# y2w-oc/CMR-Agent

Measured on AMD Instinct MI355X. Metric: registration iters/sec (KITTI 352x1216 img + 16384 pts, 1 geo forward + 10 agent steps), higher is better.
Workload: dtype f32; 1 GPU; BASELINE.json configs[1]: KittiConfig, batch 8 per GPU, 16384 pts, 352x1216 image, 10 agent steps, fp32, hash-filled weights; batch_per_gpu=8, parallelism=batch sharding, no data-path collective

## Files before the change

cmr_agent_amd/models/CMRAgent.py:

```python
import torch
import torch.nn as nn

from .. import ops
from ..utils.streams import fork_join
from . import _pack
from ._pack import Planned
from .ImageResNet import to_nhwc
from .PointNN import ConvBNReLURes1D

SLOPE = 0.01


def _mlp(sizes):
    layers = []
    for i in range(len(sizes) - 1):
        layers.append(nn.Linear(sizes[i], sizes[i + 1]))
        if i < len(sizes) - 2:
            layers.append(nn.LeakyReLU(inplace=True))
    return nn.Sequential(*layers)


class CMRAgent(Planned):
    def __init__(self, config):
        super().__init__()
# ... 47 lines not shown
                e[f:, :] = torch.eye(f, dtype=w1.dtype, device=w1.device)
                ent.update(wsca=None, wscb=e, b2=q["b2f"])
            p["s3d"].append(ent)
        return p

    def _embed_3d(self, state3d_rows, B, N):
        p = self.plan()
        layers = self.state_3d_embed
        q0 = layers[0].plan()
        r = ops.cbr_block(state3d_rows, q0["l1"][0], q0["l1"][1], q0["l2"][0], q0["b2f"], q0["sc"][0], 0.2,
                          rows_per_batch=N, want_colmax="partials")
        if r is None:
            return None
        feat, part = r
        for i, ent in enumerate(p["s3d"]):
            glue = ops.colmax_bias2(part, B, N // 32, ent["w1b"], ent["b1"], ent["wscb"], ent["b2"])
            if glue is not None:
                b1b, b2b = glue[0], glue[1]
            else:
                g = ops.colmax_partials(part, B, N // 32)
                b1b = ops.linear(g, ent["w1b"], ent["b1"])
                b2b = ops.linear(g, ent["wscb"], ent["b2"])
            last = i == 2
            r = ops.cbr_block(feat, ent["w1a"], b1b, ent["w2"], b2b, ent["wsca"], 0.2, rows_per_batch=N,
                              want_y=not last, want_colmax="partials")
            if r is None:
                return None
            feat, part = r
        return ops.colmax_partials(part, B, N // 32)

    FUSED_TAIL = True
    TAIL_T = True

    def _embed_2d(self, state2d, B, split):
        p = self.plan()
        c = 2 * self.config.embed_dim
        x = state2d
        for stage, ((wa, ba, ua), (wb, bb, ub)) in enumerate(p["convs"]):
            if stage == 0 and split is not None:
                img_src, proj, cache = split
                tag = (id(self), id(p))
                if cache.get("tag") != tag:
                    wi, bi, ui = p["conv0_img"]
                    cache["val"] = ops.conv3x3(img_src, wi, bi, c, 1, 1.0, u=ui)
                    cache["tag"] = tag
                wp, _, up = p["conv0_proj"]
                x = ops.conv3x3(proj, wp, None, c, 1, SLOPE, res=cache["val"], u=up, out_bf16=True)
            else:
                x = ops.conv3x3(x, wa, ba, c, 1, SLOPE, u=ua, out_bf16=True)
            x = ops.conv3x3(x, wb, bb, c, 1, SLOPE, pool=2 if stage < 3 else 1, u=ub, out_bf16=stage < 3)
            if stage == 3:
                kh, kw = self.config.image_H // 8, self.config.image_W // 8
                if (x.shape[1], x.shape[2]) != (kh, kw):
                    raise ValueError("state_2d is %dx%d at the global pool, config says %dx%d" % (x.shape[1], x.shape[2], kh, kw))
        return x

    def _embed_3d_any(self, state3d_rows, B, N):
        e3d = self._embed_3d(state3d_rows, B, N)
        if e3d is None:
            layers = self.state_3d_embed
            feat = layers[0].rows(state3d_rows)
            for i in (1, 2, 3):
                g = ops.colmax(feat, B, N)
                feat = layers[i].rows(feat, x2=g, div2=N)
            e3d = ops.colmax(feat, B, N)
        return e3d

    def forward_cl(self, state2d, state3d_rows, B, N, split=None):
        self._require_eval()
        e3d, e2d = fork_join(lambda: self._embed_3d_any(state3d_rows, B, N), lambda: self._embed_2d(state2d, B, split), tag="agent")
        p = self.plan()
        _, kh, kw, c = e2d.shape
        xr = e2d.view(B * kh * kw, c)
        heads = [p[name] for name in ("policy_r", "policy_t", "value")]
        if self.FUSED_TAIL and e3d.is_contiguous():
            if self.TAIL_T and p["tail_t"]:
                out, acts = ops.agent_heads_t(xr, B, kh * kw, p["c24t"], p["c26t"], e3d, [p[name + "_t"] for name in ("policy_r", "policy_t", "value")],
                                              SLOPE, actions=(self.config.num_steps, self.degree_r, self.degree_t))
# ... 72 lines not shown
```

cmr_agent_amd/models/IMGPCEnDecoder.py:

```python
import math

import torch
import torch.nn as nn

from .. import ops
from ..utils.streams import fork_join
from ._pack import Planned
from .ImageResNet import ResidualBlock
from .IMGPCEncoder import IMGPCEncoder
from .LinearAttention import LinearAttention
from .PointNN import ConvBNReLURes1D, bcl_from_rows


def position_encoding_sine_2d(d_model, h, w):
    pe = torch.zeros((d_model, h, w))
    y_pos = torch.ones((h, w)).cumsum(0).float().unsqueeze(0)
    x_pos = torch.ones((h, w)).cumsum(1).float().unsqueeze(0)
    div = torch.exp(torch.arange(0, d_model // 2, 2).float() * (-math.log(10000.0) / (d_model // 2)))[:, None, None]
    pe[0::4], pe[1::4] = torch.sin(x_pos * div), torch.cos(x_pos * div)
    pe[2::4], pe[3::4] = torch.sin(y_pos * div), torch.cos(y_pos * div)
    return pe.permute(1, 2, 0).contiguous()


class IMGPCEnDecoder(Planned):
    def __init__(self, config):
        super().__init__()
        self.config = config
        self.encoder = IMGPCEncoder(config)
        self.H_proxy = config.image_H // config.patch_size
        self.W_proxy = config.image_W // config.patch_size
        self.img_proxy_num = self.H_proxy * self.W_proxy
        self.pt_sample_num = config.pt_sample_num
        f = config.embed_dim
        self.node_fuse_convs = nn.ModuleList([ConvBNReLURes1D(2 * f, f)] +
                                             [ConvBNReLURes1D(f, f) for _ in range(config.node_fuse_res_num - 1)] +
                                             [nn.Dropout(0.1)])
        la = lambda: nn.ModuleList([LinearAttention(d_model=f, nhead=config.LA_head_num)
                                    for _ in range(config.linear_attention_num)])
        self.node_self_LA, self.pixel_to_node_LA, self.node_to_pixel_LA, self.pixel_self_LA = la(), la(), la(), la()
        self.img_fuse_convs = nn.ModuleList([ResidualBlock(2 * f, f)] +
                                            [ResidualBlock(f, f) for _ in range(config.img_fuse_res_num - 1)] +
                                            [nn.Dropout(0.1)])

    def _build_plan(self):
        return {"pe": {}}

    def _pos_table(self, h, w, device):
        cache = self.plan()["pe"]
        if (h, w) not in cache:
            cache[(h, w)] = position_encoding_sine_2d(self.config.embed_dim, h, w).to(device)
        return cache[(h, w)]

    def forward_cl(self, data_batch):
        self._require_eval()
        cl = self.encoder.forward_cl(data_batch)
        B, geo, f2 = cl["B"], cl["geo"], cl["f2"]
        _, h, w, f = f2.shape
        P = self.config.patch_size
        def fuse_nodes():
            nod = self.node_fuse_convs[0].rows(cl["node_feat"], x2=cl["pt_proxy"], idx2=cl["node2proxy_global"])
            for layer in list(self.node_fuse_convs)[1:-1]:
                nod = layer.rows(nod)
            return nod

        def fuse_pixels():
            x = ops.upsample_concat(f2, cl["img_proxy"], P)
            for i, layer in enumerate(list(self.img_fuse_convs)[:-1]):
                x = layer.forward_cl(x, post=self._pos_table(h, w, x.device) if i == 0 else None)
            return x

        nod, x = fork_join(fuse_nodes, fuse_pixels, tag="fuse")
        cl["vis_feat"] = x
        pix = x.view(B * h * w, f)
        M, L = geo.M, h * w
        for i in range(self.config.linear_attention_num):
            nod = self.pixel_to_node_LA[i].rows(nod, pix, B, M, L)
            pix = self.node_to_pixel_LA[i].rows(pix, nod, B, L, M)
            n0, p0 = nod, pix
            nod, pix = fork_join(lambda: self.node_self_LA[i].rows(n0, n0, B, M, M),
                                 lambda: self.pixel_self_LA[i].rows(p0, p0, B, L, L), tag="fine_sa")
        cl["fused_img_feat"] = pix.view(B, h, w, f)
        cl["fused_node_feat"] = nod
        cl["h"], cl["w"] = h, w
        return cl

    @staticmethod
    def publish(data_batch, cl):
        IMGPCEncoder.publish(data_batch, cl)
        data_batch['vis_feat'] = cl["vis_feat"].permute(0, 3, 1, 2)
        data_batch['fused_img_feat'] = cl["fused_img_feat"].permute(0, 3, 1, 2)
        data_batch['fused_node_feat'] = bcl_from_rows(cl["fused_node_feat"], cl["B"])

    def forward(self, data_batch):
        cl = self.forward_cl(data_batch)
        self.publish(data_batch, cl)
        data_batch['_cmr'] = cl
        return 0
```

cmr_agent_amd/models/IMGPCEncoder.py:

```python
import torch
import torch.nn as nn

from .. import ops
from ..utils.streams import fork_join, in_side_branch as streams_in_side_branch
import os
TOWERS_SWAPPED = os.environ.get("CMR_TOWERS_SWAPPED", "0") == "1"
from ._pack import Planned, device_of
from ._vit import Attention, Block, Mlp
from .ImageViT import ImageTransformer
from .PointNN import bcl_from_rows
from .PointViT import PointGeometry, PointTransformer


class IMGPCEncoder(Planned):
    def __init__(self, config):
        super().__init__()
        self.config = config
        self.pt_transformer = PointTransformer(config)
        self.img_transformer = ImageTransformer(config)
        n = config.num_ca_layer_coarse
        self.i2p_ca_layers = nn.ModuleList([Block(config) for _ in range(n)])
        self.p2i_ca_layers = nn.ModuleList([Block(config) for _ in range(n)])
        self.pt_sa_layers = nn.ModuleList([Block(config) for _ in range(n)])
        self.img_sa_layers = nn.ModuleList([Block(config) for _ in range(n)])

    def _build_plan(self):
        return {}

    def forward_cl(self, data_batch):
        dev = device_of(self)
        img = data_batch['img'].to(dev).contiguous()
        pc = data_batch['pc'].to(dev)
        node = data_batch['node'].to(dev)
        idx = data_batch['pt2node'].to(dev)
        B, Q = pc.shape[0], self.config.num_proxy

        def point_tower():
            geo = PointGeometry(pc, node, idx)
            return (geo,) + tuple(self.pt_transformer.forward_cl(geo))

        def image_tower():
            budget = ops.TOWER_CU_BUDGET if ops.CONV_BF16 else ops.TOWER_CU_BUDGET_F32
            if budget:
                give = (256 - budget) * (26.1 * pc.shape[2] / float(img.shape[2] * img.shape[3])) ** 2
                budget = 256 - 8 * int(min(256 - budget, give) / 8 + 0.5)
            if budget and budget < 256:
                with ops.conv_cu_budget(budget):
                    return self.img_transformer.forward_cl(img)
            if not ops.CONV_BF16 and ops.TOWER_SLICES_F32 > 1:
                with ops.conv_slices(ops.TOWER_SLICES_F32):
                    return self.img_transformer.forward_cl(img)
            return self.img_transformer.forward_cl(img)

        if TOWERS_SWAPPED and torch.cuda.is_available() and not streams_in_side_branch():
            (img_proxy, T, f2, f1, f0), (geo, pt_proxy, n2p, n2p_global, pt_feat, node_feat) = fork_join(image_tower, point_tower, tag="towers",
                                                                                                       main_first=False)
        else:
            (geo, pt_proxy, n2p, n2p_global, pt_feat, node_feat), (img_proxy, T, f2, f1, f0) = fork_join(point_tower, image_tower, tag="towers")
        for i in range(self.config.num_ca_layer_coarse):
            img_proxy = self.p2i_ca_layers[i].rows(img_proxy, pt_proxy, B, T, Q)
            pt_proxy = self.i2p_ca_layers[i].rows(pt_proxy, img_proxy, B, Q, T)
            ip, pp = img_proxy, pt_proxy
            pt_proxy, img_proxy = fork_join(lambda: self.pt_sa_layers[i].rows(pp, None, B, Q, Q),
                                            lambda: self.img_sa_layers[i].rows(ip, None, B, T, T), tag="coarse_sa")
        return dict(geo=geo, B=B, T=T, Q=Q, pc=pc, f2=f2, f1=f1, f0=f0, img_proxy=img_proxy, pt_proxy=pt_proxy,
                    node2proxy=n2p, node2proxy_global=n2p_global, pt_feat=pt_feat, node_feat=node_feat)

    @staticmethod
    def publish(data_batch, cl):
        B = cl["B"]
        nchw = lambda f: f.permute(0, 3, 1, 2)
        data_batch['pc_i'] = cl["pc"]
        data_batch['img_feat_2'], data_batch['img_feat_1'], data_batch['img_feat_0'] = nchw(cl["f2"]), nchw(cl["f1"]), nchw(cl["f0"])
        data_batch['node2proxy'] = cl["node2proxy"]
        data_batch['pt_feat'] = bcl_from_rows(cl["pt_feat"], B)
        data_batch['node_feat'] = bcl_from_rows(cl["node_feat"], B)
        data_batch['img_proxy'] = cl["img_proxy"].view(B, cl["T"], -1)
        data_batch['pt_proxy'] = cl["pt_proxy"].view(B, cl["Q"], -1)
        data_batch['pc'] = cl["pc"]

    def forward(self, data_batch):
        cl = self.forward_cl(data_batch)
        self.publish(data_batch, cl)
        data_batch['_cmr'] = cl
        return 0
```

cmr_agent_amd/models/ImageResNet.py:

```python
import torch
import torch.nn as nn

from .. import ops
from . import _pack
from ._pack import Planned


def _conv_bn(cin, cout, k, stride, pad):
    return [nn.Conv2d(cin, cout, k, stride, pad), nn.BatchNorm2d(cout)]


class ResidualBlock(Planned):
    SLOPE = 0.2

    def __init__(self, inchannel=3, outchannel=3, stride=1):
        super().__init__()
        assert stride in (1, 2)
        self.inchannel, self.outchannel, self.stride = inchannel, outchannel, stride
        self.conv_layers = nn.Sequential(*_conv_bn(inchannel, inchannel, 3, stride, 1),
                                         nn.LeakyReLU(self.SLOPE, inplace=True),
                                         *_conv_bn(inchannel, outchannel, 3, 1, 1))
        self.final_relu = nn.LeakyReLU(self.SLOPE, inplace=True)
        if stride == 2:
            self.shortcut = nn.Sequential(*_conv_bn(inchannel, outchannel, 3, 2, 1))
# ... 16 lines not shown
            p.update(stem=True, wa=wa.contiguous(), ba=ba.contiguous(), w3=w3.reshape(co, 27).t().contiguous(),
                     w1=w1.reshape(co, 3).t().contiguous(), bb=(b3 + b1).contiguous())
            return p
        p["stem"] = False
        p["a"] = _pack.conv9(cl[0], cl[1])
        p["b"] = _pack.conv9(cl[3], cl[4])
        if isinstance(self.shortcut, nn.Identity):
            p["sc"] = None
        elif self.shortcut[0].kernel_size == (1, 1):
            p["sc"] = ("1x1",) + _pack.lin(self.shortcut[0], self.shortcut[1])
        else:
            p["sc"] = ("3x3",) + _pack.conv9(self.shortcut[0], self.shortcut[1])
        return p

    def forward_cl(self, x, post=None, out_bf16=False):
        self._require_eval()
        p = self.plan()
        if p["stem"]:
            assert post is None
            return ops.stem_block(x, p["wa"], p["ba"], p["w3"], p["w1"], p["bb"], self.SLOPE, out_bf16=out_bf16)
        t = ops.conv3x3(x, p["a"][0], p["a"][1], self.inchannel, self.stride, self.SLOPE, u=p["a"][2],
                        out_bf16=post is None and getattr(p["b"][2], "bf16", None) is not None)
        sc = p["sc"]
        xb = x.dtype == torch.bfloat16
        if sc is None:
            res = x
        elif sc[0] == "1x1":
            B, H, W, c = x.shape
            res = ops.linear(x.view(B * H * W, c), sc[1], sc[2]).view(B, H, W, self.outchannel)
        else:
            res = ops.conv3x3(x, sc[1], sc[2], self.outchannel, 2, 1.0, u=sc[3], out_bf16=xb)
        return ops.conv3x3(t, p["b"][0], p["b"][1], self.outchannel, 1, self.SLOPE, res=res, post=post, u=p["b"][2], out_bf16=out_bf16)

    def forward(self, x):
        if self.inchannel == 3:
            return self.forward_cl(x.contiguous()).permute(0, 3, 1, 2)
        return self.forward_cl(to_nhwc(x)).permute(0, 3, 1, 2)


def to_nhwc(x):
    xp = x.permute(0, 2, 3, 1)
    if xp.is_contiguous():
        return xp
    B, C, H, W = x.shape
    return ops.transpose(x.contiguous().view(B, C, H * W)).view(B, H, W, C)


class MiniResNet(Planned):

    def __init__(self, inchannel=3, outchannel=3):
        super().__init__()
        strides = (1, 1, 2, 1, 2, 1)
        self.residual_learning = nn.ModuleList(
            [ResidualBlock(inchannel if i == 0 else outchannel, outchannel, s) for i, s in enumerate(strides)])

    def _build_plan(self):
        return {}

    def forward_cl(self, img_nchw):
        rl = self.residual_learning
        st = bool(ops.CONV_BF16 and ops.BF16_STORE and ops.BF16_CHAINS and self._bf16_served())
        x = rl[0].forward_cl(img_nchw, out_bf16=st)
        f0 = rl[1].forward_cl(x, out_bf16=st)
        f1 = rl[3].forward_cl(rl[2].forward_cl(f0, out_bf16=st), out_bf16=st)
        f2 = rl[5].forward_cl(rl[4].forward_cl(f1))
        return f2, f1, f0
# ... 13 lines not shown
```

cmr_agent_amd/ops.py:

```python
import collections
import math
import os

import numpy as np
import torch

from . import _lib

ACT_NONE, ACT_RELU, ACT_LRELU, ACT_GELU, ACT_ELU1 = 0, 1, 2, 3, 4
f32 = torch.float32
GRID_Y_MAX = 65535


def _stream():
    return torch.cuda.current_stream().cuda_stream


def _p(t):
    return None if t is None else t.data_ptr()


def _rows(t, name="tensor"):
    if t.dim() != 2 or t.stride(1) != 1 or t.dtype != f32 or not t.is_cuda:
        raise ValueError("%s must be a 2-D float32 device tensor with unit inner stride, got %s %s %s" % (
# ... 110 lines not shown

def colmax_bias2(part, B, tiles_per_batch, w1, b1, w2, b2, want_g=False):
    C = part.shape[1]
    n1, n2 = w1.shape[0], w2.shape[0]
    if COLMAX_BIAS2 == "0" or (COLMAX_BIAS2 == "fp32" and CONV_BF16) or C != 64 or n1 % 4 or n2 % 4 or not (w1.is_contiguous() and w2.is_contiguous()) or w1.shape[1] != C or w2.shape[1] != C:
        return None
    y1 = torch.empty((B, n1), dtype=f32, device=part.device)
    y2 = torch.empty((B, n2), dtype=f32, device=part.device)
    g = torch.empty((B, C), dtype=f32, device=part.device) if want_g else None
    rc = _lib.call("cmr_colmax_bias2_f32", _p(part), B, int(tiles_per_batch), C, _p(w1), _p(b1), n1, _p(w2), _p(b2), n2, _p(g), _p(y1), _p(y2), _stream(),
                   allow_unsupported=True)
    return None if rc == _lib.UNSUPPORTED else (y1, y2, g)


def layernorm64(x, gamma, beta, eps, res=None, out=None):
    _rows(x, "x")
    if out is None:
        out = torch.empty((x.shape[0], 64), dtype=f32, device=x.device)
    _lib.call("cmr_layernorm64_f32", _p(x), _ld(x), _p(gamma), _p(beta), float(eps), _p(res),
              _ld(res) if res is not None else 0, _p(out), _ld(out), x.shape[0], _stream())
    return out


CONV_BF16 = False
BF16_CHAINS = True
BF16_STORE = True
STRIDE2_FRAGS = True
WINOGRAD = True
WINO_MIN_TILES = 64


TOWER_CU_BUDGET = 160
TOWER_CU_BUDGET_F32 = 0


TOWER_SLICES_F32 = int(os.environ.get("CMR_TOWER_SLICES", "1"))


import threading

_policy = threading.local()


def _cu_budget():
    return getattr(_policy, "cu_budget", 0)


def _slices():
    return getattr(_policy, "slices", 1)


class conv_slices:

    def __init__(self, n):
        self.n = max(1, int(n))

    def __enter__(self):
        self.old, _policy.slices = _slices(), self.n

    def __exit__(self, *a):
        _policy.slices = self.old


class conv_cu_budget:

    def __init__(self, cus):
# ... 136 lines not shown
            return avgpool(conv3x3(x, w9, bias, cout, stride, slope), 2, 2)
        return y
    if out is None:
        out = torch.empty((B, ho, wo, cout), dtype=f32, device=x.device)
    _lib.call("cmr_conv3x3_nhwc_f32", _p(x), B, H, W, cin, _p(w9), _p(bias), _p(res), _p(post), _p(out), cout, stride,
              float(slope), 1, _stream())
    return out


def stem_block(img_nchw, w_a, b_a, w3, w1, b_b, slope, out_bf16=False):
    B, c, H, W = img_nchw.shape
    if c != 3 or not img_nchw.is_contiguous():
        raise ValueError("stem expects a contiguous [B,3,H,W] image")
    tmp = torch.empty((B, 6, H, W), dtype=f32, device=img_nchw.device)
    out = torch.empty((B, H, W, 64), dtype=torch.bfloat16 if out_bf16 else f32, device=img_nchw.device)
    _lib.call("cmr_stem_block_f32", _p(img_nchw), _p(w_a), _p(b_a), _p(w3), _p(w1), _p(b_b), _p(tmp), _p(out), int(out_bf16), B, H, W,
              float(slope), _stream())
    return out


def avgpool(x, kh, kw):
    B, H, W, C = x.shape
    out = torch.empty((B, H // kh, W // kw, C), dtype=f32, device=x.device)
    _lib.call("cmr_avgpool_nhwc_f32", _p(x), _p(out), B, H, W, C, kh, kw, _stream())
    return out


def upsample_concat(f, proxy_rows, scale):
    B, H, W, c1 = f.shape
    c2 = proxy_rows.shape[1]
    out = torch.empty((B, H, W, c1 + c2), dtype=f32, device=f.device)
    _lib.call("cmr_upsample_concat_f32", _p(f), _p(proxy_rows), _p(out), B, H, W, c1, c2, scale, _stream())
    return out


def patchify(x, P):
    B, H, W, C = x.shape
    out = torch.empty((B * (H // P) * (W // P), P * P * C), dtype=f32, device=x.device)
    _lib.call("cmr_patchify_nhwc_f32", _p(x), _p(out), B, H, W, C, P, _stream())
    return out


def patch_embed(x, P, w, bias, res=None, res_mod=0):
    B, H, W, C = x.shape
    n_out, K = w.shape
    rows = B * (H // P) * (W // P)
    if K % 64 == 0 and K >= 512 and (P * C) % 8 == 0 and rows <= 65536 and n_out % 4 == 0 and x.is_contiguous() and x.dtype == f32:
        out = torch.empty((rows, n_out), dtype=f32, device=x.device)
        _lib.call("cmr_patch_embed_f32", _p(x), B, H, W, C, P, _p(w), w.stride(0), _p(bias), _p(res), _ld(res) if res is not None else 0,
                  int(res_mod), _p(out), n_out, n_out, _stream())
        return out
    return linear(patchify(x, P), w, bias, res=res, res_mod=res_mod)


def transpose(x):
    b, r, c = x.shape
    if not x.is_contiguous():
        raise ValueError("transpose expects a contiguous tensor")
    out = torch.empty((b, c, r), dtype=f32, device=x.device)
    _lib.call("cmr_transpose_f32", _p(x), _p(out), b, r, c, _stream())
    return out


def mha(q, k, v, B, Tq, Tk, out=None, libm_exp=False):
    if out is None:
        out = torch.empty((B * Tq, 64), dtype=f32, device=q.device)
# ... 2045 lines not shown
```

cmr_agent_amd/runtime.py:

```python
import torch

from .environment import environment as env

INPUT_KEYS = ("img", "pc", "node", "pt2node", "K", "P")
SEGMENTED_GRAPH = __import__("os").environ.get("CMR_SEGMENTED_GRAPH_REG", "0") == "1"


class RegistrationGraph:
    def __init__(self, geo_model, agent, config, example_batch, warmup=2):
        self.geo, self.agent, self.cfg = geo_model, agent, config
        self.static_in = {k: example_batch[k].clone() for k in INPUT_KEYS if k in example_batch}
        self.graph = torch.cuda.CUDAGraph()
        side = torch.cuda.Stream()
        side.wait_stream(torch.cuda.current_stream())
        with torch.cuda.stream(side), torch.no_grad():
            for _ in range(warmup):
                self._iteration()
        torch.cuda.current_stream().wait_stream(side)
        torch.cuda.synchronize()
        if SEGMENTED_GRAPH:
            from .utils.seggraph import SegmentedGraph
            self.graph = SegmentedGraph()
            with torch.no_grad():
                self.static_pose, self.static_data = self.graph.capture(self._iteration)
        else:
            with torch.no_grad(), torch.cuda.graph(self.graph):
                self.static_pose, self.static_data = self._iteration()

    def _iteration(self):
        data = dict(self.static_in)
        self.geo(data)
        pose, target = env.init(data)
        env.to_disentangled(target, data['pc'], data=data)
        for _ in range(self.cfg.action_num):
            s2, s3 = env.observation_from_a_pose(data, pose, materialize_state_2d=False)
            r, t, v = self.agent(s2, s3)
            ar, at = self.agent.action_from_logits(r, t, deterministic=True)
            pose = env.step(ar, at, pose, self.cfg)
        self.static_last = (r, t, v)
        return pose, data

    def run(self, batch=None):
        if batch is not None:
            for k, buf in self.static_in.items():
                if batch[k].data_ptr() != buf.data_ptr():
                    buf.copy_(batch[k], non_blocking=True)
        self.graph.replay()
        return self.static_pose


class _Geo:
    def __init__(self, pc4):
        self.pc4 = pc4


class PipelinedRegistrationGraph:

    STABLE_KEYS = ("pc", "K", "P")

    TWO_GRAPHS = __import__("os").environ.get("CMR_PIPE_TWO_GRAPHS", "0") == "1"

    def __init__(self, geo_model, agent, config, example_batch, warmup=2):
        self.geo, self.agent, self.cfg = geo_model, agent, config
        self.static_in = {k: example_batch[k].clone() for k in INPUT_KEYS if k in example_batch}
        side = torch.cuda.Stream()
        side.wait_stream(torch.cuda.current_stream())
        with torch.cuda.stream(side), torch.no_grad():
            data = dict(self.static_in)
# ... 103 lines not shown
```

cmr_agent_amd/utils/workmodel.py:

```python
import torch

from .. import _lib

FP32_MFMA_PEAK = 157.3e12
HBM_PEAK = 8.0e12
RIDGE = FP32_MFMA_PEAK / HBM_PEAK
F = 4


def _linear(a):
    rows, k1, n = a["rows"], a["k1"], a["n_out"]
    k2 = a["k2"] if a["x2"] else 0
    src2 = 0
    if a["x2"]:
        src2 = rows * k2 if a["idx2"] else max(rows // max(a["div2"], 1), 1) * k2
    by = F * (rows * k1 + src2 + rows * n + n * (k1 + k2) + (rows * n if a["res"] and not a["res_mod"] else 0))
    return 2.0 * rows * (k1 + k2) * n, by


def _cbr(a):
    rows, kx, ch, co, k1 = a["rows"], a["kx"], a["ch"], a["co"], a["k1"]
    w = kx * ch + ch * co + (kx * co if a["wsc"] else 0)
    src2 = 0
    if a["x2"]:
# ... 24 lines not shown


def _vecattn(a):
    rows = a["rows"]
    if a["feat"]:
        return rows * 2.0 * (3 * 4096 + 192 + 4096 + 2 * 4096), rows * (256 + 256 + 32 + 512)
    return rows * 2.0 * (192 + 4096 + 2 * 4096), rows * (512 + 256 + 32 + 512)


WORK = {
    "cmr_linear_f32": _linear,
    "cmr_cbr_block_f32": _cbr,
    "cmr_cbr_block_bf16_f32": _cbr,
    "cmr_colmax_partials_f32": lambda a: (0, F * a["B"] * a["tiles_per_batch"] * a["C"]),
    "cmr_colmax_bias2_f32": lambda a: (2.0 * a["B"] * a["C"] * (a["n1"] + a["n2"]),
                                       F * (a["B"] * a["tiles_per_batch"] * a["C"] + (a["C"] + 1 + a["B"]) * (a["n1"] + a["n2"]))),
    "cmr_layernorm64_f32": lambda a: (0, F * a["rows"] * 64 * (3 if a["res"] else 2)),
    "cmr_conv3x3_nhwc_f32": _conv,
    "cmr_conv3x3_wino_nhwc_f32": lambda a: _conv(a, 1),
    "cmr_conv3x3_wino_stats_nhwc_f32": lambda a: (2.0 * 9 * a["Cin"] * a["Cout"] * a["B"] * a["H"] * a["W"],
                                                  F * (a["B"] * a["H"] * a["W"] * (a["Cin"] + a["Cout"]) + 9 * a["Cin"] * a["Cout"])),
    "cmr_bn_stats_from_sums_f32": lambda a: (0, F * a["parts"] * 2 * a["C"]),
    "cmr_conv3x3_wino_bnbwd_nhwc_f32": lambda a: (2.0 * 9 * a["Cin"] * a["Cout"] * a["B"] * a["H"] * a["W"],
                                                  F * (a["B"] * a["H"] * a["W"] * (a["Cin"] + 2 * a["Cout"]) + 9 * a["Cin"] * a["Cout"])),
    "cmr_bn_bwd_from_sums_f32": lambda a: (0, F * a["rows"] * a["C"] * 3),
    "cmr_conv3x3_s2_nhwc_f32": lambda a: _conv(a, 2),
    "cmr_conv3x3_bf16_nhwc_f32": _conv,
    "cmr_conv3x3_bf16io_nhwc": _conv_io,
    "cmr_conv3x3_bf16_pro_nhwc_f32": lambda a: (2.0 * 9 * a["Cin"] * a["Cout"] * a["B"] * a["H"] * a["W"],
                                                F * (a["B"] * a["H"] * a["W"] * (a["Cin"] + a["Cout"]) + 9 * a["Cin"] * a["Cout"])),
    "cmr_stem_block_f32": lambda a: (2.0 * (81 + 1728 + 192) * a["B"] * a["H"] * a["W"], a["B"] * a["H"] * a["W"] * (F * 3 + (2 if a.get("out_bf16") else F) * 64)),
    "cmr_avgpool_nhwc_f32": lambda a: (0, F * a["B"] * a["H"] * a["W"] * a["C"] * (1 + 1.0 / (a["kh"] * a["kw"]))),
    "cmr_upsample_concat_f32": lambda a: (0, F * a["B"] * a["H"] * a["W"] * (2 * a["C1"] + a["C2"] * (1 + 1.0 / a["scale"] ** 2))),
    "cmr_patchify_nhwc_f32": lambda a: (0, 2 * F * a["B"] * a["H"] * a["W"] * a["C"]),
    "cmr_transpose_f32": lambda a: (0, 2 * F * a["batch"] * a["R"] * a["Cn"]),
    "cmr_linear_rows_bf16_f32": lambda a: (2.0 * a["rows"] * a["k"] * a["n_out"], F * (a["rows"] * (a["k"] + a["n_out"] * (2 if a["res"] else 1)) + a["k"] * a["n_out"])),
    "cmr_patch_embed_f32": lambda a: (2.0 * a["B"] * (a["H"] // a["P"]) * (a["W"] // a["P"]) * a["P"] * a["P"] * a["C"] * a["n_out"],
                                     F * (a["B"] * a["H"] * a["W"] * a["C"] + a["B"] * (a["H"] // a["P"]) * (a["W"] // a["P"]) * a["n_out"] + a["P"] * a["P"] * a["C"] * a["n_out"])),
    "cmr_mha_f32": lambda a: (4.0 * a["B"] * a["Tq"] * a["Tk"] * 64, F * 64 * a["B"] * (2 * a["Tq"] + 2 * a["Tk"])),
    "cmr_mha_expf_f32": lambda a: (4.0 * a["B"] * a["Tq"] * a["Tk"] * 64, F * 64 * a["B"] * (2 * a["Tq"] + 2 * a["Tk"])),
    "cmr_mha_ln_f32": lambda a: (4.0 * a["B"] * a["Tq"] * a["Tk"] * 64 + 2.0 * 64 * a["B"] * (64 * a["Tq"] + 128 * a["Tk"]),
                                F * 64 * a["B"] * (2 * a["Tq"] + a["Tk"])),
    "cmr_la_reduce_f32": lambda a: (2.0 * a["B"] * a["S"] * 576, F * a["B"] * a["S"] * 128),
    "cmr_la_apply_f32": lambda a: (2.0 * a["B"] * a["L"] * 576, F * a["B"] * a["L"] * 128),
    "cmr_agent_heads_f32": _heads,
    "cmr_agent_heads_train_f32": _heads,
    "cmr_ln64_linear_f32": lambda a: (2.0 * 64 * (a["rows_x"] * a["n_out_x"] + (a["rows_y"] * a["n_out_y"] if a["y"] else 0)),
                                      F * (a["rows_x"] * (64 + a["n_out_x"]) + (a["rows_y"] * (64 + a["n_out_y"]) if a["y"] else 0)
                                           + 64 * (a["n_out_x"] + (a["n_out_y"] if a["y"] else 0)))),
    "cmr_ln64_linear_bf16_f32": lambda a: (2.0 * 64 * (a["rows_x"] * a["n_out_x"] + (a["rows_y"] * a["n_out_y"] if a["y"] else 0)),
                                      F * (a["rows_x"] * (64 + a["n_out_x"]) + (a["rows_y"] * (64 + a["n_out_y"]) if a["y"] else 0)
                                           + 64 * (a["n_out_x"] + (a["n_out_y"] if a["y"] else 0)))),
    "cmr_vit_out_ffn_f32": lambda a: (2.0 * a["rows"] * (4096 + 2 * 65536), F * (a["rows"] * 192 + 4096 + 2 * 65536)),
    "cmr_vit_out_ffn16_f32": lambda a: (2.0 * a["rows"] * (4096 + 2 * 65536), F * (a["rows"] * 192 + 4096 + 2 * 65536)),
    "cmr_vit_out_ffn_bf16_f32": lambda a: (2.0 * a["rows"] * (4096 + 2 * 65536), F * (a["rows"] * 192 + 4096 + 2 * 65536)),
    "cmr_la_kv_state_f32": lambda a: (2.0 * a["B"] * a["S"] * (2 * 4096 + 576), F * (a["B"] * a["S"] * 64 + 2 * 4096)),
    "cmr_la_kv_state_bf16_f32": lambda a: (2.0 * a["B"] * a["S"] * (2 * 4096 + 576), F * (a["B"] * a["S"] * 64 + 2 * 4096)),
    "cmr_la_query_layer_f32": lambda a: (2.0 * a["B"] * a["L"] * (4096 + 576 + 4096 + 16384 + 8192),
                                         F * (a["B"] * a["L"] * 128 + 2 * 4096 + 16384 + 8192)),
    "cmr_la_query_layer_bf16_f32": lambda a: (2.0 * a["B"] * a["L"] * (4096 + 576 + 4096 + 16384 + 8192),
                                         F * (a["B"] * a["L"] * 128 + 2 * 4096 + 16384 + 8192)),
    "cmr_vecattn_front_f32": _vecattn,
    "cmr_focal_metrics_f32": lambda a: (0, a["rows"] * 16),
    "cmr_circle_loss_f32": lambda a: (2.0 * a["B"] * a["n"] * a["n"] * 64, F * a["B"] * a["n"] * 128),
    "cmr_planar_to_rows_f32": lambda a: (0, F * a["B"] * a["N"] * (a["C"] + a["Cpad"])),
    "cmr_concat_rows_f32": lambda a: (0, F * a["rows"] * (2 * a["C1"] + a["C2"])),
# ... 193 lines not shown
```

include/cmr_hip.h:

```cpp
#ifndef CMR_HIP_H
#define CMR_HIP_H
#include <stdint.h>

#ifdef __cplusplus
extern "C" {
#endif

typedef struct ihipStream_t* hipStream_t;

#define CMR_OK 0
#define CMR_EINVAL -1
#define CMR_ELAUNCH -2
#define CMR_EUNSUPPORTED -3

enum { CMR_ACT_NONE = 0, CMR_ACT_RELU = 1, CMR_ACT_LRELU = 2, CMR_ACT_GELU = 3, CMR_ACT_ELU1 = 4 };


int cmr_linear_f32(const float* x1, int64_t ld1, int k1, const float* x2, int64_t ld2, int k2, const int32_t* idx2,
                   int64_t div2, const float* w, int64_t ldw, const float* bias, const float* res, int64_t ldres,
                   int64_t res_mod, float* y, int64_t ldy, int64_t rows, int n_out, int act, float act_param,
                   hipStream_t stream);
int cmr_cbr_block_f32(const float* x1, int64_t ld1, int k1, const float* x2, int64_t ld2, const int32_t* idx2,
                      int64_t div2, int kx, int ch, int co, const float* w1, const float* b1, int64_t b1_stride,
                      const float* w2, const float* b2, int64_t b2_stride, const float* wsc, float* y, int64_t ldy,
// ... 2 lines not shown
                           int64_t div2, int kx, int ch, int co, const float* w1, const float* b1, int64_t b1_stride,
                           const float* w2, const float* b2, int64_t b2_stride, const float* wsc, float* y, int64_t ldy,
                           float* colmax_part, int64_t rows, int64_t rows_per_batch, float slope, hipStream_t stream);
int cmr_colmax_partials_f32(const float* part, float* out, int B, int tiles_per_batch, int C, hipStream_t stream);
int cmr_colmax_bias2_f32(const float* part, int B, int tiles_per_batch, int C, const float* w1, const float* b1, int n1, const float* w2,
                         const float* b2, int n2, float* g, float* y1, float* y2, hipStream_t stream);

int cmr_layernorm64_f32(const float* x, int64_t ldx, const float* gamma, const float* beta, float eps, const float* res,
                        int64_t ldres, float* y, int64_t ldy, int64_t rows, hipStream_t stream);

int cmr_conv3x3_nhwc_f32(const float* x, int B, int H, int W, int Cin, const float* w, const float* bias,
                         const float* res, const float* post, float* y, int Cout, int stride, float slope, int pool,
                         hipStream_t stream);

int cmr_conv3x3_wino_nhwc_f32(const float* x, int B, int H, int W, int Cin, const float* u, const float* bias,
                              const float* res, const float* post, float* y, int Cout, float slope, int pool,
                              int cu_budget, int slices, hipStream_t stream);
int64_t cmr_conv3x3_wino_stats_parts(int B, int H, int W, int Cin, int Cout, int cu_budget, int slices);
int cmr_conv3x3_wino_stats_nhwc_f32(const float* x, int B, int H, int W, int Cin, const float* u, const float* bias, float* y, int Cout,
                                    int cu_budget, int slices, float* part, int64_t parts, hipStream_t stream);
int cmr_conv3x3_wino_bnbwd_nhwc_f32(const float* dy, int B, int H, int W, int Cin, const float* u, float* dx, int Cout, const float* bn_x,
                                    const float* bn_stat, float bn_slope, int cu_budget, int slices, float* part, int64_t parts,
                                    hipStream_t stream);
int cmr_conv3x3_s2_nhwc_f32(const float* x, int B, int H, int W, int Cin, const float* wfrag, const float* bias, const float* res,
                            const float* post, float* y, int Cout, float slope, hipStream_t stream);
int cmr_stem_block_f32(const float* x_nchw, const float* w_a, const float* b_a, const float* w3, const float* w1,
                       const float* b_b, float* tmp_nchw, void* y_nhwc, int out_bf16, int B, int H, int W, float slope,
                       hipStream_t stream);

int cmr_avgpool_nhwc_f32(const float* x, float* y, int B, int H, int W, int C, int kh, int kw, hipStream_t stream);

int cmr_upsample_concat_f32(const float* f, const float* proxy, float* out, int B, int H, int W, int C1, int C2,
                            int scale, hipStream_t stream);

int cmr_patchify_nhwc_f32(const float* x, float* out, int B, int H, int W, int C, int P, hipStream_t stream);
int cmr_patch_embed_f32(const float* x_nhwc, int B, int H, int W, int C, int P, const float* w, int64_t ldw, const float* bias,
                        const float* res, int64_t ldres, int64_t res_mod, float* y, int64_t ldy, int n_out, hipStream_t stream);
int cmr_linear_rows_bf16_f32(const float* x, int64_t ldx, int k, const float* w, int64_t ldw, const float* bias, const float* res,
                             int64_t ldres, int64_t res_mod, float* y, int64_t ldy, int64_t rows, int n_out, int act, float act_param,
                             hipStream_t stream);

int cmr_transpose_f32(const float* x, float* y, int batch, int R, int Cn, hipStream_t stream);


int cmr_mha_f32(const float* q, int64_t ldq, const float* k, int64_t ldk, const float* v, int64_t ldv, float* o,
                int64_t ldo, int B, int Tq, int Tk, hipStream_t stream);
int cmr_mha_expf_f32(const float* q, int64_t ldq, const float* k, int64_t ldk, const float* v, int64_t ldv, float* o, int64_t ldo, int B,
                     int Tq, int Tk, hipStream_t stream);
int cmr_mha_ln_f32(const float* x, int64_t ldx, const float* y, int64_t ldy, const float* gamma, const float* beta, float eps,
                   const float* wq_frag, const float* wkv_frag, const float* bq, const float* bk, const float* bv, float* o, int64_t ldo,
                   int B, int Tq, int Tk, hipStream_t stream);
int64_t cmr_la_reduce_workspace_bytes(int B, int S);
int cmr_la_reduce_f32(const float* kf, int64_t ldk, const float* v, int64_t ldv, float* kvsum, void* workspace,
                      int64_t workspace_bytes, int B, int S, hipStream_t stream);
int cmr_la_apply_f32(const float* qf, int64_t ldq, const float* kvsum, float* msg, int64_t ldm, int B, int L, int S,
                     float eps, hipStream_t stream);

int cmr_agent_heads_f32(const float* x, int B, int npix, const float* w24, const float* b24, const float* w26,
                        const float* b26, const float* e3d,
                        const float* r_w0, const float* r_b0, const float* r_w1, const float* r_b1, const float* r_w2, const float* r_b2,
                        int r_n0, int r_n1, int r_n2, float* r_out, int r_ldo,
                        const float* t_w0, const float* t_b0, const float* t_w1, const float* t_b1, const float* t_w2, const float* t_b2,
                        int t_n0, int t_n1, int t_n2, float* t_out, int t_ldo,
                        const float* v_w0, const float* v_b0, const float* v_w1, const float* v_b1, const float* v_w2, const float* v_b2,
                        int v_n0, int v_n1, int v_n2, float* v_out, int v_ldo,
                        int num_steps, int degree_r, int degree_t, int64_t* r_act, int64_t* t_act,
// ... 460 lines not shown
```

Measured before the change: 419.8 registration iters/s.

## Split first image-fuse conv into image half overlapped with matcher and proxy-class join

Result: no change. 421.9 registration iters/s (median of 6 runs) (+0.5%).

```diff
diff --git a/cmr_agent_amd/csrc/proxy_split.hip b/cmr_agent_amd/csrc/proxy_split.hip
--- /dev/null
+++ b/cmr_agent_amd/csrc/proxy_split.hip
@@ -0,0 +1,93 @@
+#include "cmr_common.h"
+
+namespace {
+
+__device__ __forceinline__ int tap_shift(int r, int k) { return (r == 0 && k == 0) ? -1 : ((r == 2 && k == 2) ? 1 : 0); }
+
+__global__ __launch_bounds__(256) void proxy_classes_kernel(const float* __restrict__ y, int64_t ldy, float* __restrict__ c, int B, int Hp,
+                                                            int Wp, int C) {
+  const unsigned c4n = (unsigned)C / 4u;
+  const unsigned total = (unsigned)B * Hp * Wp * 9u * c4n;
+  for (unsigned e = blockIdx.x * 256u + threadIdx.x; e < total; e += gridDim.x * 256u) {
+    const unsigned ch = (e % c4n) * 4u;
+    unsigned q = e / c4n;
+    const int cls = (int)(q % 9u);
+    q /= 9u;
+    const int bx = (int)(q % (unsigned)Wp), by = (int)((q / (unsigned)Wp) % (unsigned)Hp);
+    const int rc = cls / 3, qc = cls % 3;
+    f32x4 s = {0.f, 0.f, 0.f, 0.f};
+#pragma unroll
+    for (int ky = 0; ky < 3; ++ky)
+#pragma unroll
+      for (int kx = 0; kx < 3; ++kx) {
+        const int dy = tap_shift(rc, ky), dx = tap_shift(qc, kx);
+        if (by + dy < 0 || by + dy >= Hp || bx + dx < 0 || bx + dx >= Wp) continue;
+        const int64_t row = (int64_t)q + (int64_t)dy * Wp + dx;
+        s += *reinterpret_cast<const f32x4*>(y + row * ldy + (int64_t)(3 * ky + kx) * C + ch);
+      }
+    *reinterpret_cast<f32x4*>(c + (int64_t)e * 4) = s;
+  }
+}
+
+__global__ __launch_bounds__(256) void proxy_apply_kernel(const float* __restrict__ fa, const float* __restrict__ rs,
+                                                          const float* __restrict__ c, const float* __restrict__ s, int64_t lds,
+                                                          float* __restrict__ t, float* __restrict__ res, int B, int h, int w, int Ca,
+                                                          int Cs, int scale, float slope) {
+  const unsigned nva = (unsigned)Ca / 4u, nvs = (unsigned)Cs / 4u;
+  const unsigned na = (unsigned)w * nva, n = na + (unsigned)w * nvs;
+  const int Wp = w / scale, Hp = h / scale;
+  for (unsigned row = blockIdx.y; row < (unsigned)B * h; row += gridDim.y) {
+    const int yy = (int)(row % (unsigned)h), b = (int)(row / (unsigned)h);
+    const int by = yy / scale, ry = yy - by * scale;
+    const int rc = ry == 0 ? 0 : (ry == scale - 1 ? 2 : 1);
+    const int64_t tok0 = ((int64_t)b * Hp + by) * Wp;
+    const float* fa_r = fa + (int64_t)row * w * Ca;
+    const float* rs_r = rs + (int64_t)row * w * Cs;
+    float* t_r = t + (int64_t)row * w * Ca;
+    float* res_r = res + (int64_t)row * w * Cs;
+    for (unsigned i = blockIdx.x * 256u + threadIdx.x; i < n; i += gridDim.x * 256u) {
+      if (i < na) {
+        const unsigned xx = i / nva, ch = (i - xx * nva) * 4u;
+        const int bx = (int)xx / scale, rx = (int)xx - bx * scale;
+        const int cls = 3 * rc + (rx == 0 ? 0 : (rx == scale - 1 ? 2 : 1));
+        const f32x4 a = *reinterpret_cast<const f32x4*>(fa_r + (int64_t)i * 4);
+        const f32x4 k = *reinterpret_cast<const f32x4*>(c + ((tok0 + bx) * 9 + cls) * Ca + ch);
+        f32x4 v = a + k;
+#pragma unroll
+        for (int j = 0; j < 4; ++j) v[j] = v[j] > 0.f ? v[j] : v[j] * slope;
+        *reinterpret_cast<f32x4*>(t_r + (int64_t)i * 4) = v;
+      } else {
+        const unsigned j = i - na;
+        const unsigned xx = j / nvs, ch = (j - xx * nvs) * 4u;
+        const int bx = (int)xx / scale;
+        const f32x4 a = *reinterpret_cast<const f32x4*>(rs_r + (int64_t)j * 4);
+        const f32x4 k = *reinterpret_cast<const f32x4*>(s + (tok0 + bx) * lds + ch);
+        *reinterpret_cast<f32x4*>(res_r + (int64_t)j * 4) = a + k;
+      }
+    }
+  }
+}
+
+}
+
+extern "C" int cmr_proxy_conv_classes_f32(const float* y, int64_t ldy, float* c, int B, int Hp, int Wp, int C, hipStream_t stream) {
+  CMR_REQUIRE(y && c && B > 0 && Hp > 0 && Wp > 0 && C > 0 && C % 4 == 0 && ldy >= (int64_t)9 * C && ldy % 4 == 0);
+  CMR_REQUIRE(cmr_aligned16(y) && cmr_aligned16(c));
+  const int64_t total = (int64_t)B * Hp * Wp * 9 * (C / 4);
+  CMR_REQUIRE(total < ((int64_t)1 << 31));
+  hipLaunchKernelGGL(proxy_classes_kernel, dim3(cmr_fill_blocks(total, 256)), dim3(256), 0, stream, y, ldy, c, B, Hp, Wp, C);
+  return cmr_launch_status();
+}
+
+extern "C" int cmr_proxy_conv_apply_f32(const float* fa, const float* rs, const float* c, const float* s, int64_t lds, float* t, float* res,
+                                        int B, int h, int w, int Ca, int Cs, int scale, float slope, hipStream_t stream) {
+  CMR_REQUIRE(fa && rs && c && s && t && res && B > 0 && h > 0 && w > 0 && Ca > 0 && Cs > 0 && Ca % 4 == 0 && Cs % 4 == 0);
+  CMR_REQUIRE(scale >= 2 && h % scale == 0 && w % scale == 0 && lds >= Cs && lds % 4 == 0 && slope >= 0.f && slope <= 1.f);
+  CMR_REQUIRE(cmr_aligned16(fa) && cmr_aligned16(rs) && cmr_aligned16(c) && cmr_aligned16(s) && cmr_aligned16(t) && cmr_aligned16(res));
+  const int64_t per_row = (int64_t)w * ((Ca + Cs) / 4), rows = (int64_t)B * h;
+  CMR_REQUIRE(per_row < ((int64_t)1 << 31) && rows < ((int64_t)1 << 31));
+  const unsigned gx = (unsigned)((per_row + 255) / 256 < 64 ? (per_row + 255) / 256 : 64);
+  const unsigned gy = (unsigned)(rows < 65535 ? rows : 65535);
+  hipLaunchKernelGGL(proxy_apply_kernel, dim3(gx, gy), dim3(256), 0, stream, fa, rs, c, s, lds, t, res, B, h, w, Ca, Cs, scale, slope);
+  return cmr_launch_status();
+}
diff --git a/cmr_agent_amd/models/CMRAgent.py b/cmr_agent_amd/models/CMRAgent.py
--- a/cmr_agent_amd/models/CMRAgent.py
+++ b/cmr_agent_amd/models/CMRAgent.py
@@ -103,6 +103,15 @@
     FUSED_TAIL = True
     TAIL_T = True
 
+    def image_half(self, img_src, cache):
+        p = self.plan()
+        tag = (id(self), id(p))
+        if cache.get("tag") != tag:
+            wi, bi, ui = p["conv0_img"]
+            cache["val"] = ops.conv3x3(img_src, wi, bi, 2 * self.config.embed_dim, 1, 1.0, u=ui)
+            cache["tag"] = tag
+        return cache["val"]
+
     def _embed_2d(self, state2d, B, split):
         p = self.plan()
         c = 2 * self.config.embed_dim
@@ -110,11 +119,7 @@
         for stage, ((wa, ba, ua), (wb, bb, ub)) in enumerate(p["convs"]):
             if stage == 0 and split is not None:
                 img_src, proj, cache = split
-                tag = (id(self), id(p))
-                if cache.get("tag") != tag:
-                    wi, bi, ui = p["conv0_img"]
-                    cache["val"] = ops.conv3x3(img_src, wi, bi, c, 1, 1.0, u=ui)
-                    cache["tag"] = tag
+                self.image_half(img_src, cache)
                 wp, _, up = p["conv0_proj"]
                 x = ops.conv3x3(proj, wp, None, c, 1, SLOPE, res=cache["val"], u=up, out_bf16=True)
             else:
diff --git a/cmr_agent_amd/models/IMGPCEnDecoder.py b/cmr_agent_amd/models/IMGPCEnDecoder.py
--- a/cmr_agent_amd/models/IMGPCEnDecoder.py
+++ b/cmr_agent_amd/models/IMGPCEnDecoder.py
@@ -53,10 +53,21 @@
 
     def forward_cl(self, data_batch):
         self._require_eval()
-        cl = self.encoder.forward_cl(data_batch)
+        P = self.config.patch_size
+        first = self.img_fuse_convs[0]
+
+        def image_half(f2):
+            if not (ops.DECODER_SPLIT and first.split_served(f2.shape[3]) and f2.shape[1] % P == 0 and f2.shape[2] % P == 0 and P >= 2):
+                return None
+
+            def launches():
+                with ops.conv_cu_budget(ops.MATCHER_SIDE_CU_BUDGET):
+                    return first.split_image_half(f2)
+            return launches
+
+        cl = self.encoder.forward_cl(data_batch, beside_matcher=image_half)
         B, geo, f2 = cl["B"], cl["geo"], cl["f2"]
         _, h, w, f = f2.shape
-        P = self.config.patch_size
         def fuse_nodes():
             nod = self.node_fuse_convs[0].rows(cl["node_feat"], x2=cl["pt_proxy"], idx2=cl["node2proxy_global"])
             for layer in list(self.node_fuse_convs)[1:-1]:
@@ -64,9 +75,14 @@
             return nod
 
         def fuse_pixels():
-            x = ops.upsample_concat(f2, cl["img_proxy"], P)
-            for i, layer in enumerate(list(self.img_fuse_convs)[:-1]):
-                x = layer.forward_cl(x, post=self._pos_table(h, w, x.device) if i == 0 else None)
+            half = cl.pop("beside_matcher")
+            layers = list(self.img_fuse_convs)[:-1]
+            if half is not None:
+                x = first.forward_split(half, cl["img_proxy"], P, post=self._pos_table(h, w, f2.device))
+            else:
+                x = first.forward_cl(ops.upsample_concat(f2, cl["img_proxy"], P), post=self._pos_table(h, w, f2.device))
+            for layer in layers[1:]:
+                x = layer.forward_cl(x)
             return x
 
         nod, x = fork_join(fuse_nodes, fuse_pixels, tag="fuse")
diff --git a/cmr_agent_amd/models/IMGPCEncoder.py b/cmr_agent_amd/models/IMGPCEncoder.py
--- a/cmr_agent_amd/models/IMGPCEncoder.py
+++ b/cmr_agent_amd/models/IMGPCEncoder.py
@@ -27,7 +27,7 @@
     def _build_plan(self):
         return {}
 
-    def forward_cl(self, data_batch):
+    def forward_cl(self, data_batch, beside_matcher=None):
         dev = device_of(self)
         img = data_batch['img'].to(dev).contiguous()
         pc = data_batch['pc'].to(dev)
@@ -57,14 +57,24 @@
                                                                                                        main_first=False)
         else:
             (geo, pt_proxy, n2p, n2p_global, pt_feat, node_feat), (img_proxy, T, f2, f1, f0) = fork_join(point_tower, image_tower, tag="towers")
-        for i in range(self.config.num_ca_layer_coarse):
-            img_proxy = self.p2i_ca_layers[i].rows(img_proxy, pt_proxy, B, T, Q)
-            pt_proxy = self.i2p_ca_layers[i].rows(pt_proxy, img_proxy, B, Q, T)
-            ip, pp = img_proxy, pt_proxy
-            pt_proxy, img_proxy = fork_join(lambda: self.pt_sa_layers[i].rows(pp, None, B, Q, Q),
-                                            lambda: self.img_sa_layers[i].rows(ip, None, B, T, T), tag="coarse_sa")
+        def matcher(img_proxy=img_proxy, pt_proxy=pt_proxy):
+            for i in range(self.config.num_ca_layer_coarse):
+                img_proxy = self.p2i_ca_layers[i].rows(img_proxy, pt_proxy, B, T, Q)
+                pt_proxy = self.i2p_ca_layers[i].rows(pt_proxy, img_proxy, B, Q, T)
+                ip, pp = img_proxy, pt_proxy
+                pt_proxy, img_proxy = fork_join(lambda: self.pt_sa_layers[i].rows(pp, None, B, Q, Q),
+                                                lambda: self.img_sa_layers[i].rows(ip, None, B, T, T), tag="coarse_sa")
+            return img_proxy, pt_proxy
+
+        beside = None
+        job = beside_matcher(f2) if beside_matcher is not None else None
+        if job is None:
+            img_proxy, pt_proxy = matcher()
+        else:
+            beside, (img_proxy, pt_proxy) = fork_join(job, matcher, tag="matcher_side",
+                                                      main_first=not ops.MATCHER_SIDE_FIRST)
         return dict(geo=geo, B=B, T=T, Q=Q, pc=pc, f2=f2, f1=f1, f0=f0, img_proxy=img_proxy, pt_proxy=pt_proxy,
-                    node2proxy=n2p, node2proxy_global=n2p_global, pt_feat=pt_feat, node_feat=node_feat)
+                    node2proxy=n2p, node2proxy_global=n2p_global, pt_feat=pt_feat, node_feat=node_feat, beside_matcher=beside)
 
     @staticmethod
     def publish(data_batch, cl):
diff --git a/cmr_agent_amd/models/ImageResNet.py b/cmr_agent_amd/models/ImageResNet.py
--- a/cmr_agent_amd/models/ImageResNet.py
+++ b/cmr_agent_amd/models/ImageResNet.py
@@ -72,6 +72,46 @@
             res = ops.conv3x3(x, sc[1], sc[2], self.outchannel, 2, 1.0, u=sc[3], out_bf16=xb)
         return ops.conv3x3(t, p["b"][0], p["b"][1], self.outchannel, 1, self.SLOPE, res=res, post=post, u=p["b"][2], out_bf16=out_bf16)
 
+    def split_served(self, c1):
+        return (not self.training and not ops.CONV_BF16 and self.stride == 1 and 0 < c1 < self.inchannel and c1 % 8 == 0
+                and (self.inchannel - c1) % 4 == 0 and not isinstance(self.shortcut, nn.Identity) and self.shortcut[0].kernel_size == (1, 1))
+
+    def split_plan(self, c1):
+        p = self.plan()
+        if p.get("split", {}).get("c1") != c1:
+            with torch.no_grad():
+                cl = self.conv_layers
+                wa, _ = _pack.folded(cl[0], cl[1])
+                ws, bs = _pack.folded(self.shortcut[0], self.shortcut[1])
+                ws = ws.reshape(self.outchannel, self.inchannel)
+                taps = wa[:, c1:].permute(2, 3, 0, 1).reshape(9 * self.inchannel, self.inchannel - c1)
+                p["split"] = dict(c1=c1, a_img=_pack.conv9(cl[0], cl[1], cin_slice=slice(0, c1)),
+                                  proxy=torch.cat([taps, ws[:, c1:]]).contiguous(),
+                                  sc_img=(ws[:, :c1].contiguous(), bs.contiguous()))
+        return p["split"]
+
+    def split_image_half(self, f):
+        sp = self.split_plan(f.shape[3])
+        B, h, w, c1 = f.shape
+        wi, bi, ui = sp["a_img"]
+        fa = ops.conv3x3(f, wi, bi, self.inchannel, 1, 1.0, u=ui)
+        rs = ops.linear(f.view(B * h * w, c1), sp["sc_img"][0], sp["sc_img"][1])
+        return fa, rs
+
+    def split_join(self, half, proxy_rows, scale):
+        fa, rs = half
+        B, h, w, ca = fa.shape
+        sp = self.split_plan(self.inchannel - proxy_rows.shape[1])
+        y = ops.linear(proxy_rows, sp["proxy"])
+        c = ops.proxy_conv_classes(y, B, h // scale, w // scale, ca)
+        return ops.proxy_conv_apply(fa, rs, c, y[:, 9 * ca:], scale, self.SLOPE)
+
+    def forward_split(self, half, proxy_rows, scale, post=None):
+        self._require_eval()
+        t, res = self.split_join(half, proxy_rows, scale)
+        b = self.plan()["b"]
+        return ops.conv3x3(t, b[0], b[1], self.outchannel, 1, self.SLOPE, res=res, post=post, u=b[2])
+
     def forward(self, x):
         if self.inchannel == 3:
             return self.forward_cl(x.contiguous()).permute(0, 3, 1, 2)
diff --git a/cmr_agent_amd/ops.py b/cmr_agent_amd/ops.py
--- a/cmr_agent_amd/ops.py
+++ b/cmr_agent_amd/ops.py
@@ -166,6 +166,11 @@
 
 TOWER_CU_BUDGET = 160
 TOWER_CU_BUDGET_F32 = 0
+
+
+MATCHER_SIDE_CU_BUDGET = int(os.environ.get("CMR_MATCHER_SIDE_CUS", "96"))
+MATCHER_SIDE_FIRST = os.environ.get("CMR_MATCHER_SIDE_FIRST", "1") != "0"
+DECODER_SPLIT = os.environ.get("CMR_DECODER_SPLIT", "1") != "0"
 
 
 TOWER_SLICES_F32 = int(os.environ.get("CMR_TOWER_SLICES", "1"))
@@ -368,6 +373,30 @@
     out = torch.empty((B, H, W, c1 + c2), dtype=f32, device=f.device)
     _lib.call("cmr_upsample_concat_f32", _p(f), _p(proxy_rows), _p(out), B, H, W, c1, c2, scale, _stream())
     return out
+
+
+def proxy_conv_classes(y, B, Hp, Wp, C):
+    _rows(y, "y")
+    if y.shape[0] != B * Hp * Wp or y.shape[1] < 9 * C:
+        raise ValueError("proxy_conv_classes: y %s does not hold 9 x %d columns for %d x %d x %d tokens" % (tuple(y.shape), C, B, Hp, Wp))
+    c = torch.empty((B * Hp * Wp, 9, C), dtype=f32, device=y.device)
+    _lib.call("cmr_proxy_conv_classes_f32", _p(y), _ld(y), _p(c), B, Hp, Wp, C, _stream())
+    return c
+
+
+def proxy_conv_apply(fa, rs, c, s, scale, slope):
+    B, h, w, ca = fa.shape
+    _rows(rs, "rs"), _rows(s, "s")
+    cs = rs.shape[1]
+    tokens = B * (h // max(scale, 1)) * (w // max(scale, 1))
+    if (not fa.is_contiguous() or fa.dtype != f32 or not rs.is_contiguous() or rs.shape[0] != B * h * w or not c.is_contiguous()
+            or tuple(c.shape) != (tokens, 9, ca) or tuple(s.shape) != (tokens, cs)):
+        raise ValueError("proxy_conv_apply: bad operand layout")
+    t = torch.empty((B, h, w, ca), dtype=f32, device=fa.device)
+    res = torch.empty((B, h, w, cs), dtype=f32, device=fa.device)
+    _lib.call("cmr_proxy_conv_apply_f32", _p(fa), _p(rs), _p(c), _p(s), _ld(s), _p(t), _p(res), B, h, w, ca, cs, int(scale), float(slope),
+              _stream())
+    return t, res
 
 
 def patchify(x, P):
diff --git a/cmr_agent_amd/runtime.py b/cmr_agent_amd/runtime.py
--- a/cmr_agent_amd/runtime.py
+++ b/cmr_agent_amd/runtime.py
@@ -4,6 +4,8 @@
 
 INPUT_KEYS = ("img", "pc", "node", "pt2node", "K", "P")
 SEGMENTED_GRAPH = __import__("os").environ.get("CMR_SEGMENTED_GRAPH_REG", "0") == "1"
+PREFETCH_CONV0 = __import__("os").environ.get("CMR_PREFETCH_CONV0", "0") == "1"
+PREFETCH_CONV0_CUS = int(__import__("os").environ.get("CMR_PREFETCH_CONV0_CUS", "240"))
 
 
 class RegistrationGraph:
@@ -27,13 +29,29 @@
             with torch.no_grad(), torch.cuda.graph(self.graph):
                 self.static_pose, self.static_data = self._iteration()
 
+    def _first_observation(self, data):
+        pose, target = env.init(data)
+        env.to_disentangled(target, data['pc'], data=data)
+        return (pose,) + tuple(env.observation_from_a_pose(data, pose, materialize_state_2d=False))
+
     def _iteration(self):
+        from . import ops
+        from .utils.streams import fork_join
         data = dict(self.static_in)
         self.geo(data)
-        pose, target = env.init(data)
-        env.to_disentangled(target, data['pc'], data=data)
-        for _ in range(self.cfg.action_num):
-            s2, s3 = env.observation_from_a_pose(data, pose, materialize_state_2d=False)
+        cl = data.get('_cmr')
+        if PREFETCH_CONV0 and cl is not None and 'img_geo_feat' in cl and hasattr(self.agent, "image_half"):
+            pre = {}
+            def image_half():
+                with ops.conv_cu_budget(PREFETCH_CONV0_CUS):
+                    self.agent.image_half(cl['img_geo_feat'], pre)
+            _, (pose, s2, s3) = fork_join(image_half, lambda: self._first_observation(data), tag="agent_prefetch", main_first=False)
+            data['_cmr_obs'].agent_cache.update(pre)
+        else:
+            pose, s2, s3 = self._first_observation(data)
+        for i in range(self.cfg.action_num):
+            if i:
+                s2, s3 = env.observation_from_a_pose(data, pose, materialize_state_2d=False)
             r, t, v = self.agent(s2, s3)
             ar, at = self.agent.action_from_logits(r, t, deterministic=True)
             pose = env.step(ar, at, pose, self.cfg)
diff --git a/cmr_agent_amd/utils/workmodel.py b/cmr_agent_amd/utils/workmodel.py
--- a/cmr_agent_amd/utils/workmodel.py
+++ b/cmr_agent_amd/utils/workmodel.py
@@ -80,6 +80,9 @@
     "cmr_stem_block_f32": lambda a: (2.0 * (81 + 1728 + 192) * a["B"] * a["H"] * a["W"], a["B"] * a["H"] * a["W"] * (F * 3 + (2 if a.get("out_bf16") else F) * 64)),
     "cmr_avgpool_nhwc_f32": lambda a: (0, F * a["B"] * a["H"] * a["W"] * a["C"] * (1 + 1.0 / (a["kh"] * a["kw"]))),
     "cmr_upsample_concat_f32": lambda a: (0, F * a["B"] * a["H"] * a["W"] * (2 * a["C1"] + a["C2"] * (1 + 1.0 / a["scale"] ** 2))),
+    "cmr_proxy_conv_classes_f32": lambda a: (0, F * a["B"] * a["Hp"] * a["Wp"] * 18 * a["C"]),
+    "cmr_proxy_conv_apply_f32": lambda a: (0, F * (2 * a["B"] * a["h"] * a["w"] * (a["Ca"] + a["Cs"])
+                                                   + a["B"] * (a["h"] // a["scale"]) * (a["w"] // a["scale"]) * (9 * a["Ca"] + a["Cs"]))),
     "cmr_patchify_nhwc_f32": lambda a: (0, 2 * F * a["B"] * a["H"] * a["W"] * a["C"]),
     "cmr_transpose_f32": lambda a: (0, 2 * F * a["batch"] * a["R"] * a["Cn"]),
     "cmr_linear_rows_bf16_f32": lambda a: (2.0 * a["rows"] * a["k"] * a["n_out"], F * (a["rows"] * (a["k"] + a["n_out"] * (2 if a["res"] else 1)) + a["k"] * a["n_out"])),
diff --git a/include/cmr_hip.h b/include/cmr_hip.h
--- a/include/cmr_hip.h
+++ b/include/cmr_hip.h
@@ -58,6 +58,10 @@
 
 int cmr_upsample_concat_f32(const float* f, const float* proxy, float* out, int B, int H, int W, int C1, int C2,
                             int scale, hipStream_t stream);
+
+int cmr_proxy_conv_classes_f32(const float* y, int64_t ldy, float* c, int B, int Hp, int Wp, int C, hipStream_t stream);
+int cmr_proxy_conv_apply_f32(const float* fa, const float* rs, const float* c, const float* s, int64_t lds, float* t, float* res, int B,
+                             int h, int w, int Ca, int Cs, int scale, float slope, hipStream_t stream);
 
 int cmr_patchify_nhwc_f32(const float* x, float* out, int B, int H, int W, int C, int P, hipStream_t stream);
 int cmr_patch_embed_f32(const float* x_nhwc, int B, int H, int W, int C, int P, const float* w, int64_t ldw, const float* bias,
```
